# UZ-SLAMLab/ORB_SLAM2_E

Hardware: AMD Instinct MI355X
Metric: frames/s ORB extract+match (640x480, 2000 feat) (higher is better)
Workload: dtype u8; 1 GPU; 1xMI355X: batch of 64 synthetic 640x480 frames, ORB extract (2000 feat, 8 levels) + 2000x2000 brute-force Hamming match per frame; frames_per_gpu=64, global_batch=64, pipeline_contexts=3, preconditioning_steps=0, allpairs_kernel=k_match_sets_mfma_shared (FP4 matrix cores, train tiles shared through LDS), parallelism=single GPU

## Files before the change

include/orbslam_hip.h:

```cpp
#ifndef ORBSLAM_HIP_H
#define ORBSLAM_HIP_H

#include <stdint.h>

#ifdef __cplusplus
extern "C" {
#endif

enum {
    ORBX_OK = 0,
    ORBX_ERR_ARG = -1,
    ORBX_ERR_NO_DEVICE = -2,
    ORBX_ERR_HIP = -3,
    ORBX_ERR_CAPACITY = -4,
    ORBX_ERR_UNSUPPORTED = -5
};

const char *orbx_last_error(void);
int orbx_abi_version(void);


typedef struct orbx_keypoint {
    float x, y, size, angle, response;
    int32_t octave, class_id;
// ... 9 lines not shown
    int32_t trig_variant;
} orbx_params;

typedef struct orbx_extractor orbx_extractor;

int orbx_create(const orbx_params *params, orbx_extractor **out);
int orbx_destroy(orbx_extractor *ex);

int orbx_get_levels(const orbx_extractor *ex);
int orbx_get_scale_factors(const orbx_extractor *ex, float *out_nlevels);
int orbx_get_inv_scale_factors(const orbx_extractor *ex, float *out_nlevels);
int orbx_get_level_sigma2(const orbx_extractor *ex, float *out_nlevels);
int orbx_get_inv_level_sigma2(const orbx_extractor *ex, float *out_nlevels);
int orbx_get_features_per_level(const orbx_extractor *ex, int32_t *out_nlevels);
int orbx_keypoint_capacity(const orbx_extractor *ex);

int orbx_reserve(orbx_extractor *ex, int width, int height, int batch);

typedef struct {
    int32_t nlevels, keypoint_capacity, octree_nodes, cells_per_frame, sel_per_frame, fast_tile_stride, fast_lds, octree_lds, octree_kshift, reserved;
    int64_t frame_bytes, cands_per_frame;
    int32_t level_w[16], level_h[16], level_quota[16], level_nini[16], level_slots[16], level_cells[16];
} orbx_plan_info;
int orbx_plan(const orbx_params *params, int width, int height, orbx_plan_info *info);

int orbx_extract(orbx_extractor *ex, const uint8_t *image, int width, int height, int stride,
                 orbx_keypoint *kps, uint8_t *desc, int cap, int *n);

int orbx_extract_pair(orbx_extractor *left, const uint8_t *image_left, orbx_extractor *right, const uint8_t *image_right, int width,
                      int height, int stride, orbx_keypoint *kps_left, uint8_t *desc_left, int cap_left, int *n_left,
                      orbx_keypoint *kps_right, uint8_t *desc_right, int cap_right, int *n_right);

int orbx_extract_batch(orbx_extractor *ex, const uint8_t *images, int is_device,
                       int width, int height, int stride, size_t frame_stride, int batch, void *stream);
int orbx_download(orbx_extractor *ex, int frame, orbx_keypoint *kps, uint8_t *desc, int cap, int *n);
int orbx_download_batch(orbx_extractor *ex, orbx_keypoint *kps, uint8_t *desc, int32_t *counts);
int orbx_result_dev(orbx_extractor *ex, const orbx_keypoint **kps_dev, const uint8_t **desc_dev,
                    const int32_t **counts_dev, int *capacity);

int orbx_copy_results_dev(orbx_extractor *ex, orbx_keypoint *kps_dst_dev, uint8_t *desc_dst_dev,
                          int32_t *counts_dst_dev, void *stream);

int orbx_level_size(const orbx_extractor *ex, int level, int *width, int *height);
int orbx_pyramid_level(orbx_extractor *ex, int frame, int level, uint8_t *out, int out_stride);
int orbx_pyramid_level_padded(orbx_extractor *ex, int frame, int level, uint8_t *out, int out_stride);

int orbx_stereo_match(orbx_extractor *left, orbx_extractor *right, float mb, float mbf, void *stream);
int orbx_stereo_download(orbx_extractor *left, int frame, float *uRight, float *depth, int cap, int *n);
int orbx_stereo_download_batch(orbx_extractor *left, float *uRight, float *depth, int32_t *counts);

int orbx_debug_blurred_level(orbx_extractor *ex, int frame, int level, uint8_t *out, int out_stride);
int orbx_debug_level_candidates(orbx_extractor *ex, int frame, int level, float *xyr, int cap, int *n);
int orbx_debug_level_keypoints(orbx_extractor *ex, int frame, int level, orbx_keypoint *kps, int cap, int *n);

int orbx_profile_enable(orbx_extractor *ex, int on);
int orbx_profile_read(orbx_extractor *ex, int max_kinds, const char **names, double *total_ms,
                      int64_t *launches, int *nkinds);


int orbm_hamming_matrix(const uint8_t *A, int nA, const uint8_t *B, int nB, uint16_t *out);

int orbm_match_bruteforce(const uint8_t *A, int nA, const uint8_t *B, int nB,
                          int32_t *best, int32_t *second, int32_t *idx);
int orbm_match_candidates(const uint8_t *A, int nA, const uint8_t *B, int nB,
                          const int32_t *cand_off, const int32_t *cand_idx,
                          int32_t *best, int32_t *second, int32_t *idx);
typedef struct orbm_window_query {
    float u, v, r, xr;
    int32_t min_level, max_level;
} orbm_window_query;
int orbm_search_window(const orbm_window_query *queries, const uint8_t *qdesc, int nq, const orbx_keypoint *kps,
                       const uint8_t *desc, int n, const uint8_t *skip, const float *uright, float min_x, float min_y,
                       float max_x, float max_y, int init_dist, int32_t *best, int32_t *best_level, int32_t *second,
                       int32_t *second_level, int32_t *idx);

int orbm_search_fuse(const orbm_window_query *queries, const uint8_t *qdesc, int nq, const orbx_keypoint *kps, const uint8_t *desc,
                     int n, const float *uright, const float *inv_level_sigma2, int nlevels, float min_x, float min_y, float max_x,
                     float max_y, int32_t *best, int32_t *idx);

int orbm_search_projection(const orbm_window_query *queries, const uint8_t *qdesc, const float *qangle, const uint8_t *qtakes,
                           int nq, const orbx_keypoint *kps, const uint8_t *desc, int n, const uint8_t *occupied,
                           const float *uright, float min_x, float min_y, float max_x, float max_y, int th_accept, float nnratio,
                           int ratio_same_level, int check_orientation, int32_t *match_kp, int32_t *match_q, int *nmatches);

int orbm_search_for_initialization(const orbx_keypoint *kps1, const uint8_t *desc1, int n1, const orbx_keypoint *kps2,
                                   const uint8_t *desc2, int n2, float *prev_matched, float min_x, float min_y, float max_x,
                                   float max_y, int window_size, float nnratio, int check_orientation, int32_t *matches12,
                                   int *nmatches);

int orbm_search_by_bow(const int32_t *nodes1, const int32_t *off1, const int32_t *items1, int nn1, const uint8_t *valid1,
                       const uint8_t *desc1, const float *angle1, int n1, const int32_t *nodes2, const int32_t *off2,
                       const int32_t *items2, int nn2, const uint8_t *valid2, const uint8_t *desc2, const float *angle2, int n2,
                       int th, int strict_th, float nnratio, int check_orientation, int32_t *match12, int32_t *match21,
                       int *nmatches);

typedef struct orbm_camera {
    float fx, fy, cx, cy;
    int32_t min_x, max_x, min_y, max_y;
    float grid_min_x, grid_min_y, grid_max_x, grid_max_y;
} orbm_camera;
int orbm_search_by_projection_map(const orbx_keypoint *kps, const uint8_t *desc, int n, const uint8_t *has_mappoint,
                                  const float *mp_pos, const float *mp_normal, const float *mp_min_dist,
                                  const float *mp_max_dist, const uint8_t *mp_desc, int m, const double *Rcw,
                                  const double *tcw, const orbm_camera *cam, const float *scale_factors, int nlevels,
                                  float th, float nnratio, int th_reloc, int32_t *matched_mp, int *nmatches, float *proj);

// ... 230 lines not shown
```

orb_slam2_e_amd/csrc/orbx_extract.hip:

```cpp
#include <math.h>
#include <stdint.h>
#include <stdlib.h>

#include <algorithm>
#include <mutex>
#include <vector>

#include "common.h"
#include "orbx_internal.h"
#include "orbx_math.h"

using namespace orbx_detail;

namespace {

__constant__ signed char c_pattern[1024] = {
#include "orb_pattern.inc"
};

__device__ __forceinline__ int reflect101(int p, int n)
{
    if (n == 1) return 0;
    while (p < 0 || p >= n) p = p < 0 ? -p : 2 * (n - 1) - p;
    return p;
// ... 542 lines not shown
        }
    }
    if (lane == 0) cell_count[(size_t)f * cells_per_frame + c] = total;
    ORBX_PH(5, lane == 0);
    ORBX_PH(6, lane == 0);
    ORBX_PH_END(lane == 0);
}

template <int T>
__device__ void block_excl_scan2(int *a, int *b, int n, int *part, int &ta, int &tb)
{
    const int tid = threadIdx.x, lane = tid & 63, w = tid >> 6;
    __syncthreads();
    const int per = (n + T - 1) / T;
    const int lo = min(tid * per, n), hi = min(lo + per, n);
    int sa = 0, sb = 0;
    for (int i = lo; i < hi; ++i) { sa += a[i]; if (b) sb += b[i]; }
    const int ia = orbx::wave_incl_scan(sa), ib = b ? orbx::wave_incl_scan(sb) : 0;
    if (lane == 63) { part[w] = ia; part[T / 64 + w] = ib; }
    __syncthreads();
    int ba = 0, bb = 0, ga = 0, gb = 0;
#pragma unroll
    for (int i = 0; i < T / 64; ++i) {
        if (i < w) { ba += part[i]; bb += part[T / 64 + i]; }
        ga += part[i]; gb += part[T / 64 + i];
    }
    int ra = ba + ia - sa, rb = bb + ib - sb;
    for (int i = lo; i < hi; ++i) {
        const int va = a[i];
        a[i] = ra; ra += va;
        if (b) { const int vb = b[i]; b[i] = rb; rb += vb; }
    }
    ta = ga; tb = gb;
    __syncthreads();
}
template <int T>
__device__ int block_excl_scan(int *a, int n, int *part)
{
    int ta, tb;
    block_excl_scan2<T>(a, nullptr, n, part, ta, tb);
    return ta;
}

__device__ __forceinline__ void child_box(int x0, int x1, int y0, int y1, int q, int &cx0, int &cx1, int &cy0, int &cy1)
{
    const int mx = x0 + (int)ceilf((float)(x1 - x0) / 2);
    const int my = y0 + (int)ceilf((float)(y1 - y0) / 2);
    cx0 = (q & 1) ? mx : x0;
    cx1 = (q & 1) ? x1 : mx;
    cy0 = (q & 2) ? my : y0;
    cy1 = (q & 2) ? y1 : my;
}

template <int T, int KPT, int KB>
__global__ __launch_bounds__(T) void k_octree(const LevelInfo *__restrict__ L, const CellInfo *__restrict__ cells,
                                                  const int *__restrict__ cell_count, int cells_per_frame,
                                                  const uint32_t *__restrict__ cands, size_t cands_per_frame,
                                                  uint32_t *__restrict__ kpos_all, unsigned short *__restrict__ knode_all,
                                                  uint8_t *__restrict__ kq_all, size_t keys_per_frame,
                                                  uint32_t *__restrict__ sel_all, int sel_per_frame,
                                                  int *__restrict__ level_count, int *__restrict__ level_ncand,
                                                  int nlevels, int NC, int maxcells, int kcap, int kshift)
{
    extern __shared__ __align__(16) unsigned char smem[];
    int *p = reinterpret_cast<int *>(smem);
    int *part = p;          p += 2 * (T / 64);
    int *s_cell = p;        p += (maxcells + 1 + 3) & ~3;
    int *s_coff = p;        p += (maxcells + 1 + 3) & ~3;
    int *bx[2] = {p, p + NC};  p += 2 * NC;
    int *by[2] = {p, p + NC};  p += 2 * NC;
    int *cnt[2] = {p, p + NC}; p += 2 * NC;
    unsigned short *seq[2] = {reinterpret_cast<unsigned short *>(p), reinterpret_cast<unsigned short *>(p) + NC}; p += NC;
    int *cc = p;            p += 4 * NC;
    uint8_t *nne = reinterpret_cast<uint8_t *>(p), *eexp = nne + NC, *split = nne + 2 * NC; p += NC;
    unsigned short *order = reinterpret_cast<unsigned short *>(p), *bstart = order + NC;      p += NC;
    int *ebase = p;         p += NC;
    int *a1 = p;            p += NC;
    int *a2 = p;            p += NC;
    uint32_t *l_kpos = reinterpret_cast<uint32_t *>(p);                     p += kcap;
    unsigned short *l_knode = reinterpret_cast<unsigned short *>(p);        p += (kcap + 1) / 2;
    uint8_t *l_kq = reinterpret_cast<uint8_t *>(p);
    __shared__ int s_nproc;

    const int l = blockIdx.x, f = blockIdx.y, tid = threadIdx.x;
    ORBX_PH_INIT(3);
#ifdef ORBX_PHASE_TIMING
    if (tid == 0) { for (int i = 0; i < 8; ++i) ph_rec[i] = 0; ph_rec[12] = l; }
#endif
    const LevelInfo lv = L[l];
    const int N = lv.N;

    for (int c = tid; c < lv.ncells; c += T) {
        const int n = cell_count[(size_t)f * cells_per_frame + lv.cell_base + c];
        const CellInfo ci = cells[lv.cell_base + c];
        s_cell[c] = n < ci.cap ? n : ci.cap;
        s_coff[c] = ci.cand_off;
    }
    const int M = block_excl_scan<T>(s_cell, lv.ncells, part);
    if (tid == 0) s_cell[lv.ncells] = M;
    const bool in_lds = M <= kcap;
    uint32_t *kpos = in_lds ? l_kpos : kpos_all + (size_t)f * keys_per_frame + lv.key_base;
    unsigned short *knode = in_lds ? l_knode : knode_all + (size_t)f * keys_per_frame + lv.key_base;
    uint8_t *kq = in_lds ? l_kq : kq_all + (size_t)f * keys_per_frame + lv.key_base;
    uint32_t *kpos_out = kpos_all + (size_t)f * keys_per_frame + lv.key_base;
    for (int i = tid; i < NC; i += T) cnt[0][i] = 0;
    __syncthreads();
    const bool regs = M <= KPT * T;
    uint32_t kp[KPT];
    int kn[KPT], kqv[KPT];
    if (regs) {
#pragma unroll
        for (int u = 0; u < KPT; ++u) { kp[u] = 0; kn[u] = 0; kqv[u] = 0; }
#pragma unroll
        for (int h = 0; h < KPT; h += KB) {
            if (h * T >= M) break;
// ... 9 lines not shown
            }
#pragma unroll
            for (int v = 0; v < KB; ++v) {
                const int k = tid + (h + v) * T;
                if (k < M) kp[h + v] = cands[(size_t)f * cands_per_frame + s_coff[lo[v]] + (k - s_cell[lo[v]])];
            }
        }
#pragma unroll
        for (int u = 0; u < KPT; ++u) {
            const int k = tid + u * T;
            if (k < M) {
                kpos_out[k] = kp[u];
                const float x = (float)((kp[u] >> 8) & 0xfffu);
                kn[u] = (int)(x / lv.hX);
                atomicAdd(&cnt[0][kn[u]], 1);
            }
        }
    } else
    for (int k0 = tid; k0 < M; k0 += 4 * T) {
        uint32_t pk4[4];
#pragma unroll
        for (int u = 0; u < 4; ++u) {
            const int k = k0 + u * T;
            pk4[u] = 0;
            if (k < M) {
                int lo = 0, hiC = lv.ncells;
                while (hiC - lo > 1) {
                    const int mid = (lo + hiC) >> 1;
                    if (s_cell[mid] <= k) lo = mid; else hiC = mid;
                }
                pk4[u] = cands[(size_t)f * cands_per_frame + s_coff[lo] + (k - s_cell[lo])];
            }
        }
#pragma unroll
        for (int u = 0; u < 4; ++u) {
            const int k = k0 + u * T;
            if (k < M) {
                const uint32_t pk = pk4[u];
                kpos[k] = pk;
                if (in_lds) kpos_out[k] = pk;
                const float x = (float)((pk >> 8) & 0xfffu);
                const int root = (int)(x / lv.hX);
                knode[k] = (unsigned short)root;
                atomicAdd(&cnt[0][root], 1);
            }
        }
    }
    __syncthreads();
    ORBX_PHA(0, tid == 0);
#ifdef ORBX_PHASE_TIMING
    if (tid == 0) ph_rec[11] = M;
#endif
    for (int i = tid; i < lv.nIni; i += T) a1[i] = cnt[0][i] > 0 ? 1 : 0;
    int S = block_excl_scan<T>(a1, lv.nIni, part);
    for (int i = tid; i < lv.nIni; i += T) {
        if (cnt[0][i] > 0) {
            const int x0 = (int)(lv.hX * (float)i), x1 = (int)(lv.hX * (float)(i + 1));
            const int pos = a1[i];
            bx[1][pos] = x0 | (x1 << 16);
            by[1][pos] = 0 | (lv.H << 16);
            cnt[1][pos] = cnt[0][i];
            seq[1][pos] = 0;
        }
    }
    if (regs) {
#pragma unroll
        for (int u = 0; u < KPT; ++u) { if (u * T >= M) break; kn[u] = tid + u * T < M ? a1[kn[u]] : 0; }
    } else
    for (int k = tid; k < M; k += T) knode[k] = (unsigned short)a1[knode[k]];
    __syncthreads();
    ORBX_PHA(1, tid == 0);
    int cur = 1, mode = 1;

    while (true) {
        int *cx = bx[cur], *cy = by[cur], *cn = cnt[cur];
        unsigned short *cs = seq[cur];
        for (int s = tid; s < S; s += T) {
            cc[4 * s] = cc[4 * s + 1] = cc[4 * s + 2] = cc[4 * s + 3] = 0;
            split[s] = 0;
        }
        __syncthreads();
        if (regs) {
#pragma unroll
            for (int h = 0; h < KPT; h += KB) {
                if (h * T >= M) break;
                int ncn[KB], ncx[KB], ncy[KB];
#pragma unroll
                for (int v = 0; v < KB; ++v) { ncn[v] = cn[kn[h + v]]; ncx[v] = cx[kn[h + v]]; ncy[v] = cy[kn[h + v]]; }
#pragma unroll
                for (int v = 0; v < KB; ++v) {
                    const int u = h + v;
                    if (tid + u * T < M && ncn[v] > 1) {
                        const float x = (float)((kp[u] >> 8) & 0xfffu), y = (float)(kp[u] >> 20);
                        const int x0 = ncx[v] & 0xffff, x1 = ncx[v] >> 16, y0 = ncy[v] & 0xffff, y1 = ncy[v] >> 16;
                        const int mx = x0 + (int)ceilf((float)(x1 - x0) / 2);
                        const int my = y0 + (int)ceilf((float)(y1 - y0) / 2);
                        kqv[u] = (x < (float)mx ? 0 : 1) + (y < (float)my ? 0 : 2);
                        atomicAdd(&cc[4 * kn[u] + kqv[u]], 1);
                    }
                }
            }
        } else
        for (int k = tid; k < M; k += T) {
            const int s = knode[k];
            if (cn[s] > 1) {
                const uint32_t pk = kpos[k];
                const float x = (float)((pk >> 8) & 0xfffu), y = (float)(pk >> 20);
                const int x0 = cx[s] & 0xffff, x1 = cx[s] >> 16, y0 = cy[s] & 0xffff, y1 = cy[s] >> 16;
                const int mx = x0 + (int)ceilf((float)(x1 - x0) / 2);
                const int my = y0 + (int)ceilf((float)(y1 - y0) / 2);
                const int q = (x < (float)mx ? 0 : 1) + (y < (float)my ? 0 : 2);
                kq[k] = (uint8_t)q;
                atomicAdd(&cc[4 * s + q], 1);
            }
        }
        __syncthreads();
        ORBX_PHA(2, tid == 0);
        for (int s = tid; s < S; s += T) {
            int a = 0, b = 0;
            const bool cand = cn[s] > 1;
            if (cand) {
#pragma unroll
                for (int q = 0; q < 4; ++q) {
                    a += cc[4 * s + q] > 0;
                    b += cc[4 * s + q] > 1;
                }
            }
// ... 1233 lines not shown
                               ex->frame_bytes, l0, pp, (unsigned)((0x100000000ull + pp - 1) / pp), nblk_int, nb,
                               (unsigned)((0x100000000ull + nb - 1) / nb), nleft);
        } else {
            dim3 g((l0.stride / 4 + 63) / 64, (l0.h + 2 * EDGE + PYR_ROWS - 1) / PYR_ROWS, batch);
            hipLaunchKernelGGL(k_pyr_level0, g, dim3(64), 0, st, d_img, stride, frame_stride, ex->d_pyr, ex->frame_bytes, l0, aligned);
        }
        pf.stop(0, st);
    }
    const char *cmb = getenv("ORBX_PYR_CHAIN_MAX_BATCH");
    const int chain_max_batch = cmb ? atoi(cmb) : 6;
    const bool use_chain = ex->chain_tiles > 0 && batch <= chain_max_batch;
    if (use_chain) {
        pf.start(1, st);
        hipLaunchKernelGGL(k_pyr_chain, dim3(ex->chain_tiles, batch), dim3(256), ex->chain_ldsA + ex->chain_ldsB + ex->chain_ldsT + 2 * MAXL * 16, st, ex->d_pyr, ex->frame_bytes,
                           (const LevelInfo *)ex->d_lv, nl, (const ChainTile *)ex->d_chain, (const uint4 *)ex->d_chain_tabs, (const int2 *)ex->d_chain_span,
                           ex->chain_ldsA, ex->chain_ldsB);
        pf.stop(1, st);
    }
    for (int l = 1; l < nl && !use_chain; l++) {
        const LevelInfo &lv = ex->lv[l];
        const int ngi = lv.w >> 2, xlo = (PADX - EDGE) >> 2, xhi = (PADX + lv.w + EDGE - 1) >> 2;
        const int nff = ex->resize_nxi[l] ? (ngi % 64 >= 24 ? ngi / 64 + 1 : ngi / 64) : 0;
        const int nint = std::min(nff * 64, ngi);
        const int ntail = (xhi - xlo + 1) - nint;
        const int tw_shift = ntail <= 16 ? 4 : ntail <= 32 ? 5 : 6;
        const int nrg = (lv.h + 2 * EDGE + PYR_ROWS - 1) / PYR_ROWS, rpt = 64 >> tw_shift;
        const int ntw = (ntail + (1 << tw_shift) - 1) >> tw_shift;
        const int ntailw = ntw * ((nrg + rpt - 1) / rpt);
        int rpw = 1;
        while (rpw < 2 && (size_t)(nff * ((nrg + rpw - 1) / rpw) + ntailw) * batch > (size_t)ex->resident_waves) ++rpw;
        dim3 g(nff * ((nrg + rpw - 1) / rpw) + ntailw, batch);
        pf.start(1, st);
        hipLaunchKernelGGL(k_pyr_resize, g, dim3(64), 0, st, ex->d_pyr, ex->frame_bytes, ex->lv[l - 1], lv,
                           ex->d_xt + lv.xtab, ex->d_yt + lv.ytab, nff, nint, nrg, ntail, tw_shift, ntw, rpw, ex->resize_tailwin[l]);
        pf.stop(1, st);
    }
    {
        hipEvent_t e0, e1;
        pf.pair(2, &e0, &e1);
#define ORBX_FAST_LAUNCH(TS_, SS_) hipExtLaunchKernelGGL((k_fast_cells<TS_, SS_>), dim3(ex->cells_per_frame, batch), dim3(64), ex->fast_lds, st, e0, e1, 0, \
            (const uint8_t *)ex->d_pyr, ex->frame_bytes, (const LevelInfo *)ex->d_lv, (const CellInfo *)ex->d_cells, ex->d_cell_count, ex->cells_per_frame, ex->d_cands, \
            ex->cands_per_frame, ex->prm.ini_th_fast, ex->prm.min_th_fast, ex->tile_bytes, ex->sc_bytes, ex->queue_bytes)
        if (ex->TS == 52) ORBX_FAST_LAUNCH(52, 40);
        else if (ex->TS == 64) ORBX_FAST_LAUNCH(64, 64);
        else ORBX_FAST_LAUNCH(80, 80);
#undef ORBX_FAST_LAUNCH
    }
    pf.start(3, st);
    const char *owb = getenv("ORBX_OCT_WIDE_MAX_BATCH");
    if (batch <= (owb ? atoi(owb) : 6))
        hipLaunchKernelGGL((k_octree<OCT_TW, OCT_KPT * OCT_T / OCT_TW, OCT_KPT * OCT_T / OCT_TW>), dim3(nl, batch), dim3(OCT_TW), ex->oct_lds, st, ex->d_lv, ex->d_cells,
                           ex->d_cell_count, ex->cells_per_frame, ex->d_cands, ex->cands_per_frame, ex->d_kpos,
                           ex->d_knode, ex->d_kq, ex->keys_per_frame, ex->d_sel, ex->sel_per_frame, ex->d_level_count,
                           ex->d_level_ncand, nl, ex->NC, ex->maxcells, ex->oct_kcap, ex->oct_kshift);
    else
        hipLaunchKernelGGL((k_octree<OCT_T, OCT_KPT, OCT_KB>), dim3(nl, batch), dim3(OCT_T), ex->oct_lds, st, ex->d_lv, ex->d_cells,
                           ex->d_cell_count, ex->cells_per_frame, ex->d_cands, ex->cands_per_frame, ex->d_kpos,
                           ex->d_knode, ex->d_kq, ex->keys_per_frame, ex->d_sel, ex->sel_per_frame, ex->d_level_count,
                           ex->d_level_ncand, nl, ex->NC, ex->maxcells, ex->oct_kcap, ex->oct_kshift);
    pf.stop(3, st);
    pf.start(4, st);
    {
        const int S = 2 * (ex->taps[0] + ex->taps[1] + ex->taps[2]) + ex->taps[3], nt = (int)ex->tiles.size();
        const dim3 grid((unsigned)((nt + 3) / 4), batch);
        if (S > 256)
            hipLaunchKernelGGL(k_blur<true>, grid, dim3(256), 0, st, ex->d_pyr, ex->d_blur, ex->frame_bytes, ex->blur_frame_bytes, ex->d_lv, ex->d_tiles, nt,
                               ex->d_blur_frag, 128 * S * S + 32768);
        else
            hipLaunchKernelGGL(k_blur<false>, grid, dim3(256), 0, st, ex->d_pyr, ex->d_blur, ex->frame_bytes, ex->blur_frame_bytes, ex->d_lv, ex->d_tiles, nt,
                               ex->d_blur_frag, S * (128 + 128 * S) + 32768);
    }
    pf.stop(4, st);
    pf.start(5, st);
    {
        DescLevels D;
        memset(&D, 0, sizeof(D));
        int nchunks = 0;
        for (int l = 0; l < nl; l++) {
            const LevelInfo &lv = ex->lv[l];
            D.off[l] = lv.off; D.stride[l] = lv.stride; D.sel_base[l] = lv.sel_base; D.patch[l] = lv.patch; D.scale[l] = lv.scale;
            D.boff[l] = ex->boff[l]; D.bcol[l] = ex->bcol[l];
            D.chunk_base[l] = nchunks;
            nchunks += (level_slots(lv) + DESC_KPB - 1) / DESC_KPB;
        }
        for (int l = nl; l <= MAXL; l++) D.chunk_base[l] = nchunks;
        hipLaunchKernelGGL(k_describe, dim3(nchunks, batch), dim3(256), 0, st, ex->d_pyr, ex->d_blur, ex->frame_bytes, ex->blur_frame_bytes, D, nl,
                           ex->d_sel, ex->sel_per_frame, ex->d_level_count, ex->d_kps, ex->d_desc, ex->d_counts, ex->kcap, ex->prm.trig_variant,
                           batch == 1 ? ex->mirror : (uint32_t *)nullptr, ex->mirror_desc);
    }
    pf.stop(5, st);
    ORBX_HIP(hipGetLastError());
    ex->last_batch = batch;
    ex->last_stream = st;
    return ORBX_OK;
}

int orbx_profile_enable(orbx_extractor *ex, int on)
{
    if (!ex) ORBX_FAIL(ORBX_ERR_ARG, "null argument");
    static const char *names[6] = {"k_pyr_level0", "k_pyr_resize", "k_fast_cells", "k_octree", "k_blur", "k_describe"};
    for (int i = 0; i < 6; ++i) ex->prof.names[i] = names[i];
    ex->prof.reset();
    ex->prof.mask = on < 0 ? 0xffffu : (unsigned)on;
    return ORBX_OK;
}

#ifdef ORBX_PHASE_TIMING
int orbx_debug_phases(unsigned long long *out, int reset)
{
    if (out && hipMemcpyFromSymbol(out, HIP_SYMBOL(g_phase_rec), sizeof(unsigned long long) * 4 * 65536 * 16) != hipSuccess) return -1;
    if (reset) {
        void *p = nullptr;
// ... 142 lines not shown
int orbx_extract_pair(orbx_extractor *left, const uint8_t *image_left, orbx_extractor *right, const uint8_t *image_right, int width,
                      int height, int stride, orbx_keypoint *kps_left, uint8_t *desc_left, int cap_left, int *n_left,
                      orbx_keypoint *kps_right, uint8_t *desc_right, int cap_right, int *n_right)
{
    if (!left || !right || left == right || !n_left || !n_right || !image_left || !image_right || width <= 0 || height <= 0 || stride < width)
        ORBX_FAIL(ORBX_ERR_ARG, "bad arguments");
    int rc = extract_enqueue(left, image_left, width, height, stride, true);
    if (rc == ORBX_OK) rc = extract_enqueue(right, image_right, width, height, stride, true);
    if (rc != ORBX_OK) { (void)hipStreamSynchronize(left->stream); return rc; }
    rc = extract_finish(left, kps_left, desc_left, cap_left, n_left);
    const int rc2 = extract_finish(right, kps_right, desc_right, cap_right, n_right);
    return rc != ORBX_OK ? rc : rc2;
}

int orbx_result_dev(orbx_extractor *ex, const orbx_keypoint **kps, const uint8_t **desc, const int32_t **counts, int *capacity)
{
    if (!ex || !ex->d_kps) ORBX_FAIL(ORBX_ERR_ARG, "no results");
    if (kps) *kps = ex->d_kps;
    if (desc) *desc = ex->d_desc;
    if (counts) *counts = ex->d_counts;
    if (capacity) *capacity = ex->kcap;
    return ORBX_OK;
}

int orbx_copy_results_dev(orbx_extractor *ex, orbx_keypoint *kps_dst, uint8_t *desc_dst, int32_t *counts_dst, void *stream_)
{
    if (!ex || !ex->d_kps || ex->last_batch <= 0) ORBX_FAIL(ORBX_ERR_ARG, "no results");
    hipStream_t st = stream_ ? (hipStream_t)stream_ : ex->stream;
    const size_t B = (size_t)ex->last_batch;
    if (kps_dst) ORBX_HIP(hipMemcpyAsync(kps_dst, ex->d_kps, sizeof(orbx_keypoint) * ex->kcap * B, hipMemcpyDefault, st));
    if (desc_dst) ORBX_HIP(hipMemcpyAsync(desc_dst, ex->d_desc, (size_t)32 * ex->kcap * B, hipMemcpyDefault, st));
    if (counts_dst) ORBX_HIP(hipMemcpyAsync(counts_dst, ex->d_counts, sizeof(int) * B, hipMemcpyDefault, st));
    return ORBX_OK;
}

static int copy_level(orbx_extractor *ex, const uint8_t *buf, int frame, int level, uint8_t *out, int out_stride, int padded)
{
    if (!ex || !out || frame < 0 || frame >= ex->last_batch || level < 0 || level >= ex->nlevels)
        ORBX_FAIL(ORBX_ERR_ARG, "bad frame/level");
    const LevelInfo &lv = ex->lv[level];
    const int w = padded ? lv.w + 2 * EDGE : lv.w, h = padded ? lv.h + 2 * EDGE : lv.h;
    if (out_stride < w) ORBX_FAIL(ORBX_ERR_ARG, "out_stride too small");
    const uint8_t *src = buf + (size_t)frame * ex->frame_bytes + lv.off +
                         (padded ? (size_t)(PADX - EDGE) : (size_t)EDGE * lv.stride + PADX);
    ORBX_HIP(hipMemcpy2DAsync(out, out_stride, src, lv.stride, w, h, hipMemcpyDeviceToHost, ex->last_stream));
    ORBX_HIP(hipStreamSynchronize(ex->last_stream));
    return ORBX_OK;
}

int orbx_pyramid_level(orbx_extractor *ex, int frame, int level, uint8_t *out, int out_stride)
{ return copy_level(ex, ex ? ex->d_pyr : nullptr, frame, level, out, out_stride, 0); }
int orbx_pyramid_level_padded(orbx_extractor *ex, int frame, int level, uint8_t *out, int out_stride)
{ return copy_level(ex, ex ? ex->d_pyr : nullptr, frame, level, out, out_stride, 1); }
int orbx_debug_blurred_level(orbx_extractor *ex, int frame, int level, uint8_t *out, int out_stride)
{
    if (!ex || !ex->d_blur || frame < 0 || frame >= ex->last_batch || level < 0 || level >= ex->nlevels || !out)
        ORBX_FAIL(ORBX_ERR_ARG, "bad frame/level");
    const LevelInfo &lv = ex->lv[level];
    if (out_stride < lv.w) ORBX_FAIL(ORBX_ERR_ARG, "out_stride too small");
    const int nstrips = lv.stride / 16, bcol = ex->bcol[level];
    std::vector<uint8_t> strips((size_t)nstrips * bcol);
    ORBX_HIP(hipMemcpyAsync(strips.data(), ex->d_blur + (size_t)frame * ex->blur_frame_bytes + ex->boff[level], strips.size(),
                            hipMemcpyDeviceToHost, ex->last_stream));
    ORBX_HIP(hipStreamSynchronize(ex->last_stream));
    for (int y = 0; y < lv.h; ++y)
        for (int x = 0; x < lv.w; ++x) {
            const int X = PADX + x;
            out[(size_t)y * out_stride + x] = strips[(size_t)(X >> 4) * bcol + (size_t)(y + EDGE) * 16 + (X & 15)];
        }
    return ORBX_OK;
}

int orbx_debug_level_candidates(orbx_extractor *ex, int frame, int level, float *xyr, int cap, int *n)
{
    if (!ex || frame < 0 || frame >= ex->last_batch || level < 0 || level >= ex->nlevels || !n)
        ORBX_FAIL(ORBX_ERR_ARG, "bad frame/level");
    hipStream_t st = ex->last_stream;
    int M = 0;
    ORBX_HIP(hipMemcpyAsync(&M, ex->d_level_ncand + frame * ex->nlevels + level, sizeof(int), hipMemcpyDeviceToHost, st));
    ORBX_HIP(hipStreamSynchronize(st));
    *n = M;
    if (M > cap) ORBX_FAIL(ORBX_ERR_CAPACITY, "candidate buffer too small");
    std::vector<uint32_t> pk(M > 0 ? M : 1);
    if (M > 0) {
        ORBX_HIP(hipMemcpyAsync(pk.data(), ex->d_kpos + (size_t)frame * ex->keys_per_frame + ex->lv[level].key_base,
                                sizeof(uint32_t) * M, hipMemcpyDeviceToHost, st));
        ORBX_HIP(hipStreamSynchronize(st));
    }
    for (int i = 0; i < M; i++) {
        xyr[3 * i] = (float)((pk[i] >> 8) & 0xfffu);
        xyr[3 * i + 1] = (float)(pk[i] >> 20);
        xyr[3 * i + 2] = (float)(pk[i] & 0xffu);
    }
    return ORBX_OK;
}

int orbx_debug_level_keypoints(orbx_extractor *ex, int frame, int level, orbx_keypoint *kps, int cap, int *n)
{
    if (!ex || frame < 0 || frame >= ex->last_batch || level < 0 || level >= ex->nlevels || !n)
        ORBX_FAIL(ORBX_ERR_ARG, "bad frame/level");
    hipStream_t st = ex->last_stream;
    std::vector<int> lc(ex->nlevels);
    ORBX_HIP(hipMemcpyAsync(lc.data(), ex->d_level_count + frame * ex->nlevels, sizeof(int) * ex->nlevels, hipMemcpyDeviceToHost, st));
    ORBX_HIP(hipStreamSynchronize(st));
    int first = 0;
    for (int l = 0; l < level; l++) first += lc[l];
// ... 18 lines not shown
```

orb_slam2_e_amd/csrc/orbx_internal.h:

```cpp
#ifndef ORBX_INTERNAL_H
#define ORBX_INTERNAL_H

#include <stdint.h>

#include <vector>

#include "common.h"

namespace orbx_detail {

constexpr int EDGE = 19;
constexpr int PADX = 32;
constexpr int MAXL = 16;
constexpr int MIN_BORDER = EDGE - 3;
constexpr int OCT_T = 256;
constexpr int OCT_TW = 512;
constexpr int OCT_KPT = 8, OCT_KB = 4;
constexpr int OCT_MAXN = 2047;

struct LevelInfo {
    int w, h, stride, off;
    int W, H;
    int N;
    int ncells, cell_base;
    int key_base;
    int sel_base;
    int nIni;
    float hX;
    float scale;
    int patch;
    int xtab, ytab;
};

struct FastCell {
    short cw, ch, dx, dy;
    short ngx, qstep, rstep, level;
    int cand_off;
    int cap;
    int inv_ngx;
    int img_off, stride;
};
struct alignas(16) CellInfo : FastCell {
    short x0, y0;
    int pad;
};

struct ChainRect { short nx0, ny0, nw, nh, oxw0, oxw1, or0, or1; };
struct alignas(16) ChainTile { ChainRect r[MAXL]; };

struct alignas(16) BlurTile { short x0, y0, w, h; int off, stride; int boff, bcol; int pad[2]; };

}

struct orbx_extractor {
    orbx_params prm;
    int nlevels;
    float scale[orbx_detail::MAXL], inv_scale[orbx_detail::MAXL], sigma2[orbx_detail::MAXL], inv_sigma2[orbx_detail::MAXL];
    int nfeat[orbx_detail::MAXL];
    int taps[4];
    int resident_waves = 8192;
    int resize_nxi[orbx_detail::MAXL] = {};
    int resize_tailwin[orbx_detail::MAXL] = {};
    int kcap;
    int kcap_params = 0;
    size_t pin_result_off = 0;
    hipGraph_t g_graph = nullptr;
    hipGraphExec_t g_exec = nullptr;
    int g_w = 0, g_h = 0, g_stride = 0, g_seen_w = 0, g_seen_h = 0, g_seen_stride = 0;
    bool g_failed = false;

    int width = 0, height = 0, batch = 0;
    orbx_detail::LevelInfo lv[orbx_detail::MAXL];
    std::vector<orbx_detail::CellInfo> cells;
    std::vector<orbx_detail::BlurTile> tiles;
    size_t frame_bytes = 0, cands_per_frame = 0, keys_per_frame = 0;
    std::vector<orbx_detail::ChainTile> chain;
    std::vector<uint4> chain_tabs;
    std::vector<int2> chain_span;
    orbx_detail::ChainTile *d_chain = nullptr;
    uint4 *d_chain_tabs = nullptr;
    int2 *d_chain_span = nullptr;
    int chain_tiles = 0, chain_ldsA = 0, chain_ldsB = 0, chain_ldsT = 0;
    uint32_t *mirror = nullptr; int mirror_desc = 0;
    size_t blur_frame_bytes = 0;
    int boff[orbx_detail::MAXL] = {}, bcol[orbx_detail::MAXL] = {};
    int cells_per_frame = 0, sel_per_frame = 0, maxcells = 0, NC = 0;
    int TS = 0, tile_bytes = 0, SS = 0, sc_bytes = 0, fast_lds = 0, queue_bytes = 0, oct_lds = 0, oct_kcap = 0, oct_kshift = 11;

    hipStream_t stream = nullptr;
    hipStream_t last_stream = nullptr;
    hipStream_t st_stream = nullptr;
    uint8_t *d_pyr = nullptr, *d_blur = nullptr, *d_in = nullptr;
    size_t in_bytes = 0;
    orbx_detail::LevelInfo *d_lv = nullptr;
    orbx_detail::CellInfo *d_cells = nullptr;
    orbx_detail::BlurTile *d_tiles = nullptr;
    uint4 *d_blur_frag = nullptr;
    int2 *d_xt = nullptr;
    int4 *d_yt = nullptr;
    int *d_cell_count = nullptr, *d_level_count = nullptr, *d_level_ncand = nullptr, *d_counts = nullptr;
    uint32_t *d_cands = nullptr, *d_kpos = nullptr, *d_sel = nullptr;
    unsigned short *d_knode = nullptr;
    uint8_t *d_kq = nullptr, *d_desc = nullptr;
    orbx_keypoint *d_kps = nullptr;
    int last_batch = 0;
    uint8_t *h_pin = nullptr;
    size_t pin_bytes = 0;
    unsigned *d_st_key = nullptr;
    void *d_st_rk = nullptr;
    int *d_st_rowoff = nullptr, *d_st_items = nullptr;
    uint8_t *h_st_pin = nullptr; size_t st_pin_bytes = 0;
    float *d_uright = nullptr, *d_depth = nullptr, *d_st_scale = nullptr;
    int *d_st_sad = nullptr, *d_st_nvalid = nullptr;
    int st_batch = 0, st_cap = 0;
    bool st_valid = false;
    orbx::KernelProfiler prof;
    hipEvent_t order_ev = nullptr, reader_ev = nullptr;
    hipStream_t reader_stream = nullptr;
    bool reader_pending = false;
};

namespace orbx_detail {
orbx_extractor *order_after_producer(const void *ptr, hipStream_t st);
void reader_done(orbx_extractor *ex, hipStream_t st);
}

#endif
```

orb_slam2_e_amd/extractor.py:

```python
import ctypes as C

import numpy as np

from ._lib import check, lib, ptr as _p

KP_DTYPE = np.dtype([("x", "<f4"), ("y", "<f4"), ("size", "<f4"), ("angle", "<f4"),
                     ("response", "<f4"), ("octave", "<i4"), ("class_id", "<i4")])


class _Params(C.Structure):
    _fields_ = [("nfeatures", C.c_int32), ("scale_factor", C.c_float), ("nlevels", C.c_int32),
                ("ini_th_fast", C.c_int32), ("min_th_fast", C.c_int32), ("blur_variant", C.c_int32), ("trig_variant", C.c_int32)]




class ORBextractor:
    def __init__(self, nfeatures, scaleFactor, nlevels, iniThFAST, minThFAST, blur_variant=0, trig_variant=0):
        self._L = lib()
        self._h = C.c_void_p()
        prm = _Params(nfeatures, scaleFactor, nlevels, iniThFAST, minThFAST, blur_variant, trig_variant)
        check(self._L.orbx_create(C.byref(prm), C.byref(self._h)))
        self.nlevels = nlevels
        self.capacity = self._L.orbx_keypoint_capacity(self._h)
# ... 70 lines not shown

    def download(self, frame):
        kps = np.zeros(self.capacity, KP_DTYPE)
        desc = np.zeros((self.capacity, 32), np.uint8)
        n = C.c_int(0)
        check(self._L.orbx_download(self._h, frame, _p(kps), _p(desc), self.capacity, C.byref(n)))
        return kps[:n.value].copy(), desc[:n.value].copy()

    def download_batch(self):
        B = self._last_B
        kps = np.zeros((B, self.capacity), KP_DTYPE); desc = np.zeros((B, self.capacity, 32), np.uint8)
        cnt = np.zeros(B, np.int32)
        check(self._L.orbx_download_batch(self._h, _p(kps), _p(desc), _p(cnt)))
        return kps, desc, cnt

    def result_dev(self):
        kps, desc, cnt, cap = C.c_void_p(), C.c_void_p(), C.c_void_p(), C.c_int()
        check(self._L.orbx_result_dev(self._h, C.byref(kps), C.byref(desc), C.byref(cnt), C.byref(cap)))
        return kps.value, desc.value, cnt.value, cap.value

    def level_size(self, level):
        w, h = C.c_int(), C.c_int()
        check(self._L.orbx_level_size(self._h, level, C.byref(w), C.byref(h)))
        return w.value, h.value

    def pyramid_level(self, frame, level, padded=False):
        w, h = self.level_size(level)
        if padded:
            w, h = w + 38, h + 38
        out = np.zeros((h, w), np.uint8)
        fn = self._L.orbx_pyramid_level_padded if padded else self._L.orbx_pyramid_level
        check(fn(self._h, frame, level, _p(out), w))
        return out

    def blurred_level(self, frame, level):
        w, h = self.level_size(level)
        out = np.zeros((h, w), np.uint8)
        check(self._L.orbx_debug_blurred_level(self._h, frame, level, _p(out), w))
        return out

    def level_candidates(self, frame, level):
        w, h = self.level_size(level)
        cap = w * h // 4 + 16
        out = np.zeros((cap, 3), np.float32)
        n = C.c_int(0)
        check(self._L.orbx_debug_level_candidates(self._h, frame, level, _p(out), cap, C.byref(n)))
        return out[:n.value].copy()

    def level_keypoints(self, frame, level):
        out = np.zeros(self.capacity, KP_DTYPE)
        n = C.c_int(0)
        check(self._L.orbx_debug_level_keypoints(self._h, frame, level, _p(out), self.capacity, C.byref(n)))
        return out[:n.value].copy()


class _ExtractPlan(C.Structure):
    _fields_ = [(n, C.c_int32) for n in ("nlevels", "keypoint_capacity", "octree_nodes", "cells_per_frame", "sel_per_frame", "fast_tile_stride",
                                         "fast_lds", "octree_lds", "octree_kshift", "reserved")] + \
               [("frame_bytes", C.c_int64), ("cands_per_frame", C.c_int64)] + \
               [(n, C.c_int32 * 16) for n in ("level_w", "level_h", "level_quota", "level_nini", "level_slots", "level_cells")]


def plan(nfeatures, scaleFactor, nlevels, iniThFAST, minThFAST, width, height):
    L = lib()
    prm = _Params(nfeatures, scaleFactor, nlevels, iniThFAST, minThFAST, 0)
    info = _ExtractPlan()
    check(L.orbx_plan(C.byref(prm), int(width), int(height), C.byref(info)))
    out = {}
    for n, t in _ExtractPlan._fields_:
        v = getattr(info, n)
        out[n] = list(v)[:info.nlevels] if n.startswith("level_") else v
    return out


def extract_pair(left, right, image_left, image_right):
    il = np.ascontiguousarray(image_left); ir = np.ascontiguousarray(image_right)
    assert il.dtype == np.uint8 and il.ndim == 2 and il.shape == ir.shape and ir.dtype == np.uint8
    h, w = il.shape
    left._reserve(w, h, 1); right._reserve(w, h, 1)
    out = []
    for e in (left, right):
        out.append((np.zeros(e.capacity, KP_DTYPE), np.zeros((e.capacity, 32), np.uint8), C.c_int(0)))
    (kl, dl, nl), (kr, dr, nr) = out
    check(left._L.orbx_extract_pair(left._h, _p(il), right._h, _p(ir), w, h, il.strides[0], _p(kl), _p(dl), left.capacity, C.byref(nl),
                                    _p(kr), _p(dr), right.capacity, C.byref(nr)))
    left._shape = right._shape = (h, w)
    return (kl[:nl.value].copy(), dl[:nl.value].copy()), (kr[:nr.value].copy(), dr[:nr.value].copy())


def stereo_match_batch(left, right, mb, mbf, stream=None):
    check(left._L.orbx_stereo_match(left._h, right._h, mb, mbf, stream))


def stereo_download_batch(left):
    B = left._last_B
    u = np.zeros((B, left.capacity), np.float32); d = np.zeros((B, left.capacity), np.float32); c = np.zeros(B, np.int32)
    check(left._L.orbx_stereo_download_batch(left._h, _p(u), _p(d), _p(c)))
    return u, d, c


def ComputeStereoMatches(left, right, mb, mbf, frame=0):
    L = left._L
    check(L.orbx_stereo_match(left._h, right._h, mb, mbf, None))
    u = np.zeros(left.capacity, np.float32); d = np.zeros(left.capacity, np.float32)
    n = C.c_int(0)
    check(L.orbx_stereo_download(left._h, frame, _p(u), _p(d), left.capacity, C.byref(n)))
# ... 2 lines not shown
```

Measured before the change: 279,600 frames/s.

## Build top octree levels directly via per-key quadrant binning in k_octree

Adds a direct path to the octree distribution kernel. Each keypoint computes its quadrant path down to OCT_RMAX levels and atomically counts into per-depth bins held in LDS, reusing the kpos scratch space. A scan over those bins then works out how many split rounds the iterative loop would perform and materialises the resulting node set in one pass, so the per-round split-and-sync iterations for the shallow levels are skipped. It is enabled by default, adds atomics and extra LDS scan work, and must reproduce the iterative split order exactly.

```diff
diff --git a/include/orbslam_hip.h b/include/orbslam_hip.h
--- a/include/orbslam_hip.h
+++ b/include/orbslam_hip.h
@@ -85,6 +85,7 @@
 int orbx_debug_blurred_level(orbx_extractor *ex, int frame, int level, uint8_t *out, int out_stride);
 int orbx_debug_level_candidates(orbx_extractor *ex, int frame, int level, float *xyr, int cap, int *n);
 int orbx_debug_level_keypoints(orbx_extractor *ex, int frame, int level, orbx_keypoint *kps, int cap, int *n);
+int orbx_debug_octree_direct(orbx_extractor *ex, int on);
 
 int orbx_profile_enable(orbx_extractor *ex, int on);
 int orbx_profile_read(orbx_extractor *ex, int max_kinds, const char **names, double *total_ms,
diff --git a/orb_slam2_e_amd/csrc/orbx_extract.hip b/orb_slam2_e_amd/csrc/orbx_extract.hip
--- a/orb_slam2_e_amd/csrc/orbx_extract.hip
+++ b/orb_slam2_e_amd/csrc/orbx_extract.hip
@@ -618,6 +618,13 @@
     cy1 = (q & 2) ? y1 : my;
 }
 
+__device__ __forceinline__ int oct_bin_off(int d) { return ((1 << (2 * d)) - 1) / 3; }
+__device__ __forceinline__ int oct_bin(int nr, int root, int d, int path)
+{
+    const int m = (1 << (2 * d)) - 1;
+    return nr * oct_bin_off(d) + (((d & 1) ? nr - 1 - root : root) << (2 * d)) + (path ^ (0x333 & m));
+}
+
 template <int T, int KPT, int KB>
 __global__ __launch_bounds__(T) void k_octree(const LevelInfo *__restrict__ L, const CellInfo *__restrict__ cells,
                                                   const int *__restrict__ cell_count, int cells_per_frame,
@@ -626,7 +633,7 @@
                                                   uint8_t *__restrict__ kq_all, size_t keys_per_frame,
                                                   uint32_t *__restrict__ sel_all, int sel_per_frame,
                                                   int *__restrict__ level_count, int *__restrict__ level_ncand,
-                                                  int nlevels, int NC, int maxcells, int kcap, int kshift)
+                                                  int nlevels, int NC, int maxcells, int kcap, int kshift, int direct)
 {
     extern __shared__ __align__(16) unsigned char smem[];
     int *p = reinterpret_cast<int *>(smem);
@@ -742,7 +749,15 @@
     if (tid == 0) ph_rec[11] = M;
 #endif
     for (int i = tid; i < lv.nIni; i += T) a1[i] = cnt[0][i] > 0 ? 1 : 0;
-    int S = block_excl_scan<T>(a1, lv.nIni, part);
+    int S = __builtin_amdgcn_readfirstlane(block_excl_scan<T>(a1, lv.nIni, part));
+    int rmax = 0;
+    int *const bins = reinterpret_cast<int *>(l_kpos);
+    if (direct && regs && S > 0) {
+        const int room = kcap + (kcap + 1) / 2 + (kcap + 3) / 4;
+        for (rmax = OCT_RMAX; rmax > 0 && 2 * lv.nIni * oct_bin_off(rmax + 1) > room; --rmax) {}
+    }
+    int *const pre = bins + lv.nIni * oct_bin_off(rmax + 1);
+    const int nb = S * oct_bin_off(rmax + 1);
     for (int i = tid; i < lv.nIni; i += T) {
         if (cnt[0][i] > 0) {
             const int x0 = (int)(lv.hX * (float)i), x1 = (int)(lv.hX * (float)(i + 1));
@@ -751,18 +766,111 @@
             by[1][pos] = 0 | (lv.H << 16);
             cnt[1][pos] = cnt[0][i];
             seq[1][pos] = 0;
-        }
-    }
+            if (rmax) bins[pos] = cnt[0][i];
+        }
+    }
+    if (rmax)
+        for (int i = S + tid; i < nb; i += T) bins[i] = 0;
     if (regs) {
 #pragma unroll
         for (int u = 0; u < KPT; ++u) { if (u * T >= M) break; kn[u] = tid + u * T < M ? a1[kn[u]] : 0; }
     } else
     for (int k = tid; k < M; k += T) knode[k] = (unsigned short)a1[knode[k]];
     __syncthreads();
+    int cur = 1, mode = 1;
+    if (rmax) {
+#pragma unroll
+        for (int u = 0; u < KPT; ++u) {
+            if (u * T >= M) break;
+            if (tid + u * T < M) {
+                const int r0 = kn[u], rx = bx[1][r0], ry = by[1][r0];
+                const int x = (int)((kp[u] >> 8) & 0xfffu), y = (int)(kp[u] >> 20);
+                int x0 = rx & 0xffff, x1 = rx >> 16, y0 = ry & 0xffff, y1 = ry >> 16, path = 0;
+                for (int d = 1; d <= rmax; ++d) {
+                    const int mx = x0 + ((x1 - x0 + 1) >> 1), my = y0 + ((y1 - y0 + 1) >> 1);
+                    const bool qx = x >= mx, qy = y >= my;
+                    path = 4 * path + (qx ? 1 : 0) + (qy ? 2 : 0);
+                    x0 = qx ? mx : x0; x1 = qx ? x1 : mx;
+                    y0 = qy ? my : y0; y1 = qy ? y1 : my;
+                    atomicAdd(&bins[oct_bin(S, r0, d, path)], 1);
+                }
+                kqv[u] = path;
+            }
+        }
+        __syncthreads();
+        for (int i = tid; i < nb; i += T) {
+            int d = 0;
+            while (i >= S * oct_bin_off(d + 1)) ++d;
+            const int rel = i - S * oct_bin_off(d), m = (1 << (2 * d)) - 1;
+            const int rk = rel >> (2 * d), path = (rel & m) ^ (0x333 & m), r0 = (d & 1) ? S - 1 - rk : rk;
+            const int c = bins[i];
+            bool ok = c > 0;
+            for (int a = 0; a < d; ++a) ok = ok && bins[oct_bin(S, r0, a, path >> (2 * (d - a)))] > 1;
+            pre[i] = ok ? 1 | ((c > 1 ? 1 : 0) << 16) : 0;
+        }
+        const int tot = __builtin_amdgcn_readfirstlane(block_excl_scan<T>(pre, nb, part));
+        const auto upto_v = [&](int d) { return d > rmax ? tot : pre[S * oct_bin_off(d)]; };
+        const auto upto = [&](int d) { return __builtin_amdgcn_readfirstlane(upto_v(d)); };
+        int R = 0, leaves = 0, Sr = S;
+        while (true) {
+            const int t = upto(R + 1) - upto(R);
+            if ((t >> 16) == 0) { mode = 0; break; }
+            if (R == rmax) break;
+            leaves += (t & 0xffff) - (t >> 16);
+            ++R;
+            const int t2 = upto(R + 1) - upto(R), Sn = (t2 & 0xffff) + leaves;
+            const bool fin = Sn >= N || Sn == Sr;
+            Sr = Sn;
+            if (fin) { mode = 0; break; }
+            if (Sn + 3 * (t2 >> 16) > N) { mode = 2; break; }
+        }
+        if (R > 0) {
+            const int tR = upto(R + 1) - upto(R), nR = tR & 0xffff, eR = tR >> 16;
+            for (int i = tid; i < S * oct_bin_off(R + 1); i += T) {
+                int d = 0;
+                while (i >= S * oct_bin_off(d + 1)) ++d;
+                const int rel = i - S * oct_bin_off(d), m = (1 << (2 * d)) - 1;
+                const int rk = rel >> (2 * d), path = (rel & m) ^ (0x333 & m), r0 = (d & 1) ? S - 1 - rk : rk;
+                const int pi = pre[i], fl = (i + 1 < nb ? pre[i + 1] : tot) - pi, before = pi - upto_v(d);
+                int pos = -1, sq = 0;
+                if (fl & 0xffff) {
+                    if (d == R) {
+                        pos = before & 0xffff;
+                        sq = (fl >> 16) ? eR - 1 - (before >> 16) : 0;
+                    } else if ((fl >> 16) == 0) {
+                        pos = nR + (before & 0xffff) - (before >> 16);
+                        for (int j = d + 1; j < R; ++j) { const int tj = upto_v(j + 1) - upto_v(j); pos += (tj & 0xffff) - (tj >> 16); }
+                    }
+                }
+                if (pos >= 0) {
+                    const int rx = bx[1][r0], ry = by[1][r0];
+                    int x0 = rx & 0xffff, x1 = rx >> 16, y0 = ry & 0xffff, y1 = ry >> 16;
+                    for (int j = 1; j <= d; ++j) child_box(x0, x1, y0, y1, (path >> (2 * (d - j))) & 3, x0, x1, y0, y1);
+                    bx[0][pos] = x0 | (x1 << 16);
+                    by[0][pos] = y0 | (y1 << 16);
+                    cnt[0][pos] = bins[i];
+                    seq[0][pos] = (unsigned short)sq;
+                }
+                bins[i] = pos;
+            }
+            __syncthreads();
+#pragma unroll
+            for (int u = 0; u < KPT; ++u) {
+                if (u * T >= M) break;
+                if (tid + u * T < M) {
+                    const int r0 = kn[u];
+                    for (int d = 0; d <= R; ++d) {
+                        const int v = bins[oct_bin(S, r0, d, kqv[u] >> (2 * (rmax - d)))];
+                        if (v >= 0) kn[u] = v;
+                    }
+                }
+            }
+            S = Sr; cur = 0;
+        }
+    }
     ORBX_PHA(1, tid == 0);
-    int cur = 1, mode = 1;
-
-    while (true) {
+
+    while (mode != 0) {
         int *cx = bx[cur], *cy = by[cur], *cn = cnt[cur];
         unsigned short *cs = seq[cur];
         for (int s = tid; s < S; s += T) {
@@ -2102,12 +2210,12 @@
         hipLaunchKernelGGL((k_octree<OCT_TW, OCT_KPT * OCT_T / OCT_TW, OCT_KPT * OCT_T / OCT_TW>), dim3(nl, batch), dim3(OCT_TW), ex->oct_lds, st, ex->d_lv, ex->d_cells,
                            ex->d_cell_count, ex->cells_per_frame, ex->d_cands, ex->cands_per_frame, ex->d_kpos,
                            ex->d_knode, ex->d_kq, ex->keys_per_frame, ex->d_sel, ex->sel_per_frame, ex->d_level_count,
-                           ex->d_level_ncand, nl, ex->NC, ex->maxcells, ex->oct_kcap, ex->oct_kshift);
+                           ex->d_level_ncand, nl, ex->NC, ex->maxcells, ex->oct_kcap, ex->oct_kshift, ex->oct_direct);
     else
         hipLaunchKernelGGL((k_octree<OCT_T, OCT_KPT, OCT_KB>), dim3(nl, batch), dim3(OCT_T), ex->oct_lds, st, ex->d_lv, ex->d_cells,
                            ex->d_cell_count, ex->cells_per_frame, ex->d_cands, ex->cands_per_frame, ex->d_kpos,
                            ex->d_knode, ex->d_kq, ex->keys_per_frame, ex->d_sel, ex->sel_per_frame, ex->d_level_count,
-                           ex->d_level_ncand, nl, ex->NC, ex->maxcells, ex->oct_kcap, ex->oct_kshift);
+                           ex->d_level_ncand, nl, ex->NC, ex->maxcells, ex->oct_kcap, ex->oct_kshift, ex->oct_direct);
     pf.stop(3, st);
     pf.start(4, st);
     {
@@ -2356,6 +2464,13 @@
 { return copy_level(ex, ex ? ex->d_pyr : nullptr, frame, level, out, out_stride, 0); }
 int orbx_pyramid_level_padded(orbx_extractor *ex, int frame, int level, uint8_t *out, int out_stride)
 { return copy_level(ex, ex ? ex->d_pyr : nullptr, frame, level, out, out_stride, 1); }
+int orbx_debug_octree_direct(orbx_extractor *ex, int on)
+{
+    if (!ex) ORBX_FAIL(ORBX_ERR_ARG, "null handle");
+    ex->oct_direct = on ? 1 : 0;
+    return ORBX_OK;
+}
+
 int orbx_debug_blurred_level(orbx_extractor *ex, int frame, int level, uint8_t *out, int out_stride)
 {
     if (!ex || !ex->d_blur || frame < 0 || frame >= ex->last_batch || level < 0 || level >= ex->nlevels || !out)
diff --git a/orb_slam2_e_amd/csrc/orbx_internal.h b/orb_slam2_e_amd/csrc/orbx_internal.h
--- a/orb_slam2_e_amd/csrc/orbx_internal.h
+++ b/orb_slam2_e_amd/csrc/orbx_internal.h
@@ -16,6 +16,7 @@
 constexpr int OCT_T = 256;
 constexpr int OCT_TW = 512;
 constexpr int OCT_KPT = 8, OCT_KB = 4;
+constexpr int OCT_RMAX = 4;
 constexpr int OCT_MAXN = 2047;
 
 struct LevelInfo {
@@ -86,6 +87,7 @@
     int boff[orbx_detail::MAXL] = {}, bcol[orbx_detail::MAXL] = {};
     int cells_per_frame = 0, sel_per_frame = 0, maxcells = 0, NC = 0;
     int TS = 0, tile_bytes = 0, SS = 0, sc_bytes = 0, fast_lds = 0, queue_bytes = 0, oct_lds = 0, oct_kcap = 0, oct_kshift = 11;
+    int oct_direct = 1;
 
     hipStream_t stream = nullptr;
     hipStream_t last_stream = nullptr;
diff --git a/orb_slam2_e_amd/extractor.py b/orb_slam2_e_amd/extractor.py
--- a/orb_slam2_e_amd/extractor.py
+++ b/orb_slam2_e_amd/extractor.py
@@ -146,6 +146,9 @@
         n = C.c_int(0)
         check(self._L.orbx_debug_level_keypoints(self._h, frame, level, _p(out), self.capacity, C.byref(n)))
         return out[:n.value].copy()
+
+    def octree_direct(self, on):
+        check(self._L.orbx_debug_octree_direct(self._h, 1 if on else 0))
 
 
 class _ExtractPlan(C.Structure):
```

Result: no change. 282,000 frames/s, median of 2 (+0.9%).
